# genjax-community/genjax

Measured on AMD Instinct MI355X. Metric: particle_steps_per_sec, higher is better.
Workload: dtype f32; 1 GPU; gmm_c8_d16 ImportanceK: propagate+reweight+LSE, systematic resample, gather (BASELINE.json configs[1]); k_particles_per_gpu=1048576, k_particles_total=1048576, rng_stream=flat, exchange=none

## Files before the change

### genjax_amd/csrc/gjx_resample.hip

```cpp
#include <math.h>
#include <string.h>

#include "gjx_device.h"
#include "gjx_host.h"
#include "gjx_scan.h"
#include "gjx_tile.h"

namespace gjx {

struct PickPair {
  float v;
  int32_t i;
};

GJX_DEV void pick_better(float& v, int32_t& i, float ov, int32_t oi) {
  if (ov > v || (ov == v && oi < i)) { v = ov; i = oi; }
}

template <int RNG>
__global__ __launch_bounds__(256) void k_pick_partial(const float* logw, int64_t K, int64_t offset, const float* lse,
                                                     key2 key, PickPair* partials) {
  __shared__ float rv[4];
  __shared__ int32_t ri[4];
  const float l = lse[2];
  float bv = -INFINITY;
  int32_t bi = 0x7FFFFFFF;
  for (int64_t i = (int64_t)blockIdx.x * 256 + threadIdx.x; i < K; i += (int64_t)gridDim.x * 256) {
    const uint64_t gi = (uint64_t)(offset + i);
    uint32_t bits;
    if (RNG == GJX_RNG_JAX32) {
      const key2 h = fold_in64(key, gi);
      bits = h.a ^ h.b;
    } else {
      const key2 h = fold_in64(key, gi >> 1);
      bits = (gi & 1u) ? h.b : h.a;
    }
    const float v = (logw[i] - l) + gumbel_from_bits(bits);
    pick_better(bv, bi, v, (int32_t)gi);
  }
#pragma unroll
  for (int o = 32; o > 0; o >>= 1) {
    const float ov = __shfl_xor(bv, o, 64);
    const int32_t oi = __shfl_xor(bi, o, 64);
    pick_better(bv, bi, ov, oi);
  }
  if ((threadIdx.x & 63) == 0) { rv[threadIdx.x >> 6] = bv; ri[threadIdx.x >> 6] = bi; }
  __syncthreads();
  if (threadIdx.x == 0) {
    for (int w = 1; w < 4; ++w) pick_better(bv, bi, rv[w], ri[w]);
    partials[blockIdx.x] = PickPair{bv, bi};
  }
}

__global__ __launch_bounds__(256) void k_pick_finish(const PickPair* partials, int n, PickPair* out) {
  __shared__ float rv[4];
  __shared__ int32_t ri[4];
  float bv = -INFINITY;
  int32_t bi = 0x7FFFFFFF;
  for (int t = threadIdx.x; t < n; t += 256) pick_better(bv, bi, partials[t].v, partials[t].i);
#pragma unroll
  for (int o = 32; o > 0; o >>= 1) {
    const float ov = __shfl_xor(bv, o, 64);
    const int32_t oi = __shfl_xor(bi, o, 64);
    pick_better(bv, bi, ov, oi);
  }
  if ((threadIdx.x & 63) == 0) { rv[threadIdx.x >> 6] = bv; ri[threadIdx.x >> 6] = bi; }
  __syncthreads();
  if (threadIdx.x == 0) {
    for (int w = 1; w < 4; ++w) pick_better(bv, bi, rv[w], ri[w]);
    *out = PickPair{bv, bi};
  }
}

template <int RNG>
__global__ __launch_bounds__(256) void k_trials_lse_pick(const float* logw, int64_t K, int64_t offset, key2 key, int want_pick, float log_k,
                                                        float* lse_out, int32_t* pick_out) {
  __shared__ float red[8];
  __shared__ float rv[4];
  __shared__ int32_t ri[4];
  const int64_t t = blockIdx.x;
  const float* lw = logw + t * K;
  float m = -INFINITY;
  for (int64_t i = threadIdx.x; i < K; i += 256) m = fmaxf(m, lw[i]);
  m = wave_max(m);
  if ((threadIdx.x & 63) == 0) red[threadIdx.x >> 6] = m;
  __syncthreads();
  const float bm = fmaxf(fmaxf(red[0], red[1]), fmaxf(red[2], red[3]));
  float sm = 0.0f;
  if (bm > -INFINITY)
    for (int64_t i = threadIdx.x; i < K; i += 256) sm += fast_exp(lw[i] - bm);
  sm = wave_sum(sm);
  if ((threadIdx.x & 63) == 0) red[4 + (threadIdx.x >> 6)] = sm;
  __syncthreads();
  const float bs = (red[4] + red[5]) + (red[6] + red[7]);
  const float l = bm > -INFINITY ? bm + fast_log(bs) : -INFINITY;
  if (threadIdx.x == 0) {
    float* o = lse_out + 4 * t;
    o[0] = bm; o[1] = bs; o[2] = l; o[3] = l - log_k;
  }
  if (!want_pick) return;
  float bv = -INFINITY;
  int32_t bi = 0x7FFFFFFF;
  for (int64_t i = threadIdx.x; i < K; i += 256) {
    const uint64_t gi = (uint64_t)(offset + t * K + i);
    uint32_t bits;
    if (RNG == GJX_RNG_JAX32) {
      const key2 h = fold_in64(key, gi);
      bits = h.a ^ h.b;
    } else {
      const key2 h = fold_in64(key, gi >> 1);
      bits = (gi & 1u) ? h.b : h.a;
    }
    pick_better(bv, bi, (lw[i] - l) + gumbel_from_bits(bits), (int32_t)gi);
  }
#pragma unroll
  for (int o = 32; o > 0; o >>= 1) {
    const float ov = __shfl_xor(bv, o, 64);
    const int32_t oi = __shfl_xor(bi, o, 64);
    pick_better(bv, bi, ov, oi);
  }
  if ((threadIdx.x & 63) == 0) { rv[threadIdx.x >> 6] = bv; ri[threadIdx.x >> 6] = bi; }
  __syncthreads();
  if (threadIdx.x == 0) {
    for (int w = 1; w < 4; ++w) pick_better(bv, bi, rv[w], ri[w]);
    pick_out[t] = bi == 0x7FFFFFFF ? (int32_t)(offset + t * K) : bi;
  }
}

__global__ __launch_bounds__(256) void k_wsum_blocks(const float* x, int64_t K, int is_log, const float* lse,
                                                    int n_partials, float* lse_out, float log_k_total,
                                                    uint64_t* block_sums) {
  __shared__ uint64_t red[4];
  __shared__ float fred[8];
  float sm;
  const float mx = block_ref_max(is_log, lse, n_partials, fred, &sm);
  if (is_log == 2 && lse_out && blockIdx.x == 0 && threadIdx.x == 0) {
    const float l = mx > -INFINITY ? mx + logf(sm) : -INFINITY;
    lse_out[0] = mx; lse_out[1] = sm; lse_out[2] = l; lse_out[3] = l - log_k_total;
  }
  const int64_t base = (int64_t)blockIdx.x * kScanTile + (int64_t)threadIdx.x * kScanItems;
  uint64_t s = 0;
#pragma unroll
  for (int k = 0; k < kScanItems; ++k)
    if (base + k < K) s += weight_q(x, base + k, is_log, mx);
  s = wave_sum_u64(s);
  if ((threadIdx.x & 63) == 0) red[threadIdx.x >> 6] = s;
  __syncthreads();
  if (threadIdx.x == 0) block_sums[blockIdx.x] = red[0] + red[1] + red[2] + red[3];
}

__global__ __launch_bounds__(256) void k_wscan_write(const float* x, int64_t K, int is_log, const float* lse,
                                                    int n_partials, const uint64_t* block_sums, uint64_t* cum,
                                                    uint64_t* base_total) {
  __shared__ uint64_t wsum[4];
  __shared__ uint64_t red[4];
  __shared__ float fred[8];
  const float mx = block_ref_max(is_log, lse, n_partials, fred, nullptr);
  const int64_t base = (int64_t)blockIdx.x * kScanTile + (int64_t)threadIdx.x * kScanItems;
  uint64_t pre = 0;
  for (int t = threadIdx.x; t < (int)blockIdx.x; t += 256) pre += block_sums[t];
  pre = wave_sum_u64(pre);
  if ((threadIdx.x & 63) == 0) red[threadIdx.x >> 6] = pre;
  uint64_t q[kScanItems];
  uint64_t s = 0;
#pragma unroll
  for (int k = 0; k < kScanItems; ++k) {
    q[k] = (base + k < K) ? weight_q(x, base + k, is_log, mx) : 0;
    s += q[k];
    q[k] = s;
  }
  uint64_t inc = wave_scan_u64(s);
  if ((threadIdx.x & 63) == 63) wsum[threadIdx.x >> 6] = inc;
  __syncthreads();
  uint64_t off = red[0] + red[1] + red[2] + red[3] + inc - s;
  for (int w = 0; w < (int)(threadIdx.x >> 6); ++w) off += wsum[w];
#pragma unroll
  for (int k = 0; k < kScanItems; ++k)
    if (base + k < K) cum[base + k] = off + q[k];
  if (blockIdx.x == gridDim.x - 1 && threadIdx.x == 255) {
    base_total[0] = 0;
    base_total[1] = off + s;
  }
}

GJX_DEV int64_t upper_search(const uint64_t* __restrict__ cum, int64_t K, uint64_t t) {
  int64_t lo = 0, hi = K - 1;
  while (lo < hi) {
    const int64_t mid = (lo + hi) >> 1;
    if (cum[mid] > t) hi = mid; else lo = mid + 1;
  }
  return lo;
}

GJX_DEV int64_t upper_search_in(const uint64_t* __restrict__ cum, int64_t lo, int64_t hi, uint64_t t) {
  while (lo < hi) {
    const int64_t mid = (lo + hi) >> 1;
    if (cum[mid] > t) hi = mid; else lo = mid + 1;
  }
  return lo;
}

template <bool GATHER>
__global__ __launch_bounds__(256) void k_systematic_expand(const uint64_t* __restrict__ cum, int64_t K,
                                                          const uint64_t* base_total, double u, int64_t N_total,
                                                          int64_t out_begin, int64_t n_out, int32_t* ancestors,
                                                          const float* __restrict__ src, int64_t src_stride, int rows,
                                                          float* __restrict__ dst, int64_t dst_stride,
                                                          const int64_t* range_dev = nullptr) {
  constexpr int kOwn = 8;
  if (range_dev) {
    out_begin = range_dev[0];
    const int64_t n = range_dev[1];
    n_out = n < n_out ? n : n_out;
  }
  __shared__ int n_heavy;
  __shared__ int32_t h_i[256];
  __shared__ int64_t h_lo[256], h_hi[256];
  if (threadIdx.x == 0) n_heavy = 0;
  __syncthreads();
  const int64_t i = (int64_t)blockIdx.x * 256 + threadIdx.x;
  const uint64_t base = base_total[0], total = base_total[1];
  const double step = (double)total / (double)N_total;
  const double inv_step = (double)N_total / (double)total;
  const bool in = i < K && total > 0;
  const uint64_t c_cur = in ? base + cum[i] : 0;
  const int64_t j_cur = in ? slots_below(c_cur, u, step, inv_step, total, N_total) : 0;
  int64_t j_prev = __shfl_up((long long)j_cur, 1, 64);
  uint64_t c_prev = __shfl_up((unsigned long long)c_cur, 1, 64);
  if ((threadIdx.x & 63) == 0) {
    c_prev = base + ((in && i > 0) ? cum[i - 1] : 0);
    j_prev = in ? slots_below(c_prev, u, step, inv_step, total, N_total) : 0;
  }
  if (in) {
    if (c_cur > c_prev) {
      int64_t lo = j_prev - out_begin;
      int64_t hi = j_cur - out_begin;
      lo = lo < 0 ? 0 : lo;
      hi = hi > n_out ? n_out : hi;
      if (hi - lo > kOwn) {
        const int h = atomicAdd(&n_heavy, 1);
        h_i[h] = (int32_t)i; h_lo[h] = lo; h_hi[h] = hi;
      } else if (hi > lo) {
        if (ancestors) for (int64_t j = lo; j < hi; ++j) ancestors[j] = (int32_t)i;
        if (GATHER) {
          for (int r = 0; r < rows; ++r) {
            const float v = src[(int64_t)r * src_stride + i];
            for (int64_t j = lo; j < hi; ++j) dst[(int64_t)r * dst_stride + j] = v;
          }
        }
      }
    }
  }
  __syncthreads();
  const int nh = n_heavy;
  for (int h = 0; h < nh; ++h) {
    const int32_t pi = h_i[h];
    const int64_t lo = h_lo[h], hi = h_hi[h];
    if (ancestors) for (int64_t j = lo + threadIdx.x; j < hi; j += 256) ancestors[j] = pi;
    if (GATHER) {
      for (int r = 0; r < rows; ++r) {
        const float v = src[(int64_t)r * src_stride + pi];
        for (int64_t j = lo + threadIdx.x; j < hi; j += 256) dst[(int64_t)r * dst_stride + j] = v;
      }
    }
  }
}

template <int ITEMS>
__global__ __launch_bounds__(256) void k_resample_fused(const float* __restrict__ x, int64_t K, int mode,
                                                       const float* lse, int n_partials, float* lse_out,
                                                       float log_k_total, double u, int64_t N, int32_t* ancestors,
                                                       uint64_t* cum_out, uint64_t* base_total_out,
                                                       unsigned long long* agg, unsigned* ctrl) {
  __shared__ float fred[8];
  __shared__ ScanSmem sm;
  unsigned epoch;
  const unsigned long long tag = grid_tag(ctrl, &epoch);
  const int64_t i0 = ((int64_t)blockIdx.x * 256 + threadIdx.x) * ITEMS;
  float xv[ITEMS];
#pragma unroll
  for (int k = 0; k < ITEMS; ++k) xv[k] = (i0 + k < K) ? x[i0 + k] : 0.0f;
  float sm_sum;
  const float mx = block_ref_max(mode, lse, n_partials, fred, &sm_sum);
  if (mode == 2 && lse_out && blockIdx.x == 0 && threadIdx.x == 0) {
    const float l = mx > -INFINITY ? mx + logf(sm_sum) : -INFINITY;
    lse_out[0] = mx; lse_out[1] = sm_sum; lse_out[2] = l; lse_out[3] = l - log_k_total;
  }
  tile_scan_expand<ITEMS, false>(xv, mode, mx, i0, K, u, N, ancestors, cum_out, base_total_out, agg, tag, ctrl, epoch, true, sm);
}

constexpr int kGatherMaxTiles = 1024;

template <int ITEMS>
__global__ __launch_bounds__(256) void k_resample_gather(const float* __restrict__ x, int64_t K, int mode,
                                                        const float* lse, int n_partials, float* lse_out,
                                                        float log_k_total, double u, const float* __restrict__ src,
                                                        int64_t src_stride, int rows, float* __restrict__ dst,
                                                        int64_t dst_stride, int32_t* ancestors,
                                                        unsigned long long* agg, unsigned* ctrl,
                                                        unsigned long long* timeline) {
#define GJX_STAMP(n) do { if (timeline && threadIdx.x == 0) timeline[blockIdx.x * 8 + (n)] = __builtin_amdgcn_s_memrealtime(); } while (0)
  GJX_STAMP(0);
  constexpr int TILE = 256 * ITEMS;
  __shared__ float fred[8];
  __shared__ uint64_t wsum[4];
  __shared__ uint64_t P[kGatherMaxTiles + 1];
  constexpr int CH = 3;
  __shared__ uint64_t cumL[CH * TILE];
  __shared__ uint64_t s_wtot[CH][4];
  __shared__ int s_range[2];
  unsigned epoch;
  const unsigned long long tag = grid_tag(ctrl, &epoch);
  const int nb = (int)gridDim.x;
  const int lane = threadIdx.x & 63, wid = threadIdx.x >> 6;
  const int64_t i0 = ((int64_t)blockIdx.x * 256 + threadIdx.x) * ITEMS;
  auto load_tile = [&](int64_t p0, float (&v)[ITEMS]) {
    if (ITEMS == 4 && p0 + 4 <= K) {
      const float4 q4 = *(const float4*)(x + p0);
      v[0] = q4.x; v[1] = q4.y; v[2] = q4.z; v[3] = q4.w;
    } else {
#pragma unroll
      for (int k = 0; k < ITEMS; ++k) v[k] = (p0 + k < K) ? x[p0 + k] : 0.0f;
    }
  };
  const int w0 = (int)blockIdx.x - 1;
  float xv[ITEMS], xn[2][ITEMS];
  load_tile(i0, xv);
  float sm_sum;
  const float mx = block_ref_max(mode, lse, n_partials, fred, &sm_sum);
  if (mode == 2 && lse_out && blockIdx.x == 0 && threadIdx.x == 0) {
    const float l = mx > -INFINITY ? mx + logf(sm_sum) : -INFINITY;
    lse_out[0] = mx; lse_out[1] = sm_sum; lse_out[2] = l; lse_out[3] = l - log_k_total;
  }
  uint64_t qown[ITEMS], sown = 0, incown;
  {
#pragma unroll
    for (int k = 0; k < ITEMS; ++k) { sown += (i0 + k < K) ? weight_q(xv, k, mode, mx) : 0; qown[k] = sown; }
    incown = wave_scan_u64(sown);
    if (lane == 63) { wsum[wid] = incown; s_wtot[1][wid] = incown; }
    __syncthreads();
    if (threadIdx.x == 0) grid_publish(agg, tag, wsum[0] + wsum[1] + wsum[2] + wsum[3]);
  }
  GJX_STAMP(1);
#pragma unroll
  for (int c = 0; c < 2; ++c) {
    const int tc = w0 + 2 * c;
#pragma unroll
    for (int k = 0; k < ITEMS; ++k) xn[c][k] = 0.0f;
    if (tc >= 0 && tc < nb) load_tile((int64_t)tc * TILE + (int64_t)threadIdx.x * ITEMS, xn[c]);
  }
  {
    uint64_t qn[2][ITEMS], sn[2], incn[2];
#pragma unroll
    for (int c = 0; c < 2; ++c) {
      const int tc = w0 + 2 * c;
      const bool on = tc >= 0 && tc < nb;
      const int64_t p0 = (int64_t)tc * TILE + (int64_t)threadIdx.x * ITEMS;
      sn[c] = 0;
#pragma unroll
      for (int k = 0; k < ITEMS; ++k) { sn[c] += (on && p0 + k < K) ? weight_q(xn[c], k, mode, mx) : 0; qn[c][k] = sn[c]; }
    }
#pragma unroll
    for (int c = 0; c < 2; ++c) incn[c] = wave_scan_u64(sn[c]);
    if (lane == 63) { s_wtot[0][wid] = incn[0]; s_wtot[2][wid] = incn[1]; }
    __syncthreads();
#pragma unroll
    for (int c = 0; c < 3; ++c) {
      uint64_t base = c == 1 ? incown - sown : incn[c >> 1] - sn[c >> 1];
      for (int w = 0; w < wid; ++w) base += s_wtot[c][w];
#pragma unroll
      for (int k = 0; k < ITEMS; ++k) cumL[c * TILE + threadIdx.x * ITEMS + k] = base + (c == 1 ? qown[k] : qn[c >> 1][k]);
    }
  }
  grid_gather(agg, tag, ctrl, [&](int b, unsigned long long val) { P[b + 1] = val; });
  if (threadIdx.x == 0) P[0] = 0;
  __syncthreads();
  GJX_STAMP(2);
  prefix_in_place<256>(P, nb, wsum, NoShift{});
  const uint64_t total = P[nb];
  GJX_STAMP(6);
  if (blockIdx.x == 0 && threadIdx.x == 0) {
    __hip_atomic_store(&ctrl[0], epoch + 1u, __ATOMIC_RELAXED, __HIP_MEMORY_SCOPE_AGENT);
    if (total == 0) __hip_atomic_fetch_or(&ctrl[2], kStatusZeroTotal, __ATOMIC_RELAXED, __HIP_MEMORY_SCOPE_AGENT);
  }
  int32_t anc[ITEMS];
#pragma unroll
  for (int k = 0; k < ITEMS; ++k) anc[k] = (int32_t)((i0 + k < K) ? i0 + k : 0);
  if (total > 0) {
    const double step = (double)total / (double)K;
    uint64_t T[ITEMS];
    int tile[ITEMS], kpos[ITEMS];
#pragma unroll
    for (int k = 0; k < ITEMS; ++k) {
      const int64_t j = (i0 + k < K) ? i0 + k : K - 1;
      T[k] = comb_threshold(j, u, step, total);
    }
    source_tiles<ITEMS>(P, nb, (int)blockIdx.x, T, tile);
    if (timeline) { asm volatile("" :: "v"(tile[0]), "v"(tile[ITEMS - 1])); GJX_STAMP(7); }
    if (threadIdx.x == 0) s_range[0] = tile[0];
    if (threadIdx.x == 255) s_range[1] = tile[ITEMS - 1];
    __syncthreads();
    const int tmin = s_range[0], ntiles = s_range[1] - tmin + 1;
    int pos[ITEMS];
    const uint64_t* cm[ITEMS];
    uint64_t Tr[ITEMS];
#pragma unroll
    for (int k = 0; k < ITEMS; ++k) Tr[k] = T[k] - P[tile[k]];
    if (tmin >= w0 && s_range[1] <= w0 + 2) {
      GJX_STAMP(3);
#pragma unroll
      for (int k = 0; k < ITEMS; ++k) cm[k] = cumL + (tile[k] - w0) * TILE;
      rank_in_tiles<TILE, ITEMS>(cm, Tr, pos);
#pragma unroll
      for (int k = 0; k < ITEMS; ++k) anc[k] = (int32_t)((int64_t)tile[k] * TILE + pos[k]);
    } else {
#pragma unroll
    for (int k = 0; k < ITEMS; ++k) kpos[k] = tile[k] - tmin;
    auto next_live = [&](int at) { while (at < ntiles && P[tmin + at + 1] == P[tmin + at]) ++at; return at; };
    GJX_STAMP(3);
    float nv[CH][ITEMS];
#pragma unroll
    for (int c = 0; c < CH; ++c)
      if (c < ntiles) load_tile((int64_t)(tmin + c) * TILE + (int64_t)threadIdx.x * ITEMS, nv[c]);
    for (int idx = 0; idx < ntiles;) {
      const int nidx = next_live(idx + CH);
      rescan_round<256, TILE, ITEMS, CH>(cumL, &s_wtot[0][0], [&](int c, int o, uint64_t (&q)[ITEMS]) {
        const bool on = idx + c < ntiles;
        const int64_t p0 = (int64_t)(tmin + idx + c) * TILE + o;
        if (on) {
#pragma unroll
          for (int k = 0; k < ITEMS; ++k) q[k] = (p0 + k < K) ? weight_q(nv[c], k, mode, mx) : 0;
        }
        if (nidx + c < ntiles) load_tile((int64_t)(tmin + nidx + c) * TILE + o, nv[c]);
        return on;
      }, [] {});
      bool mine[ITEMS];
#pragma unroll
      for (int k = 0; k < ITEMS; ++k) {
        mine[k] = kpos[k] >= idx && kpos[k] < idx + CH;
        cm[k] = cumL + (mine[k] ? (kpos[k] - idx) * TILE : 0);
      }
      rank_in_tiles<TILE, ITEMS>(cm, Tr, pos);
#pragma unroll
      for (int k = 0; k < ITEMS; ++k)
        if (mine[k]) anc[k] = (int32_t)((int64_t)tile[k] * TILE + pos[k]);
      idx = nidx;
    }
    }
  }
  GJX_STAMP(4);
#pragma unroll
  for (int k = 0; k < ITEMS; ++k) anc[k] = max(0, min(anc[k], (int32_t)(K - 1)));
  const bool whole = i0 + ITEMS <= K;
  if (ancestors) {
    if (ITEMS == 4 && whole) *(int4*)(ancestors + i0) = make_int4(anc[0], anc[1], anc[2], anc[3]);
    else {
#pragma unroll
      for (int k = 0; k < ITEMS; ++k) if (i0 + k < K) ancestors[i0 + k] = anc[k];
    }
  }
  const bool vec = ITEMS == 4 && whole && (dst_stride & 3) == 0 && (((uintptr_t)dst) & 15) == 0;
  if (vec) {
#pragma unroll 4
    for (int r = 0; r < rows; ++r) {
      const float* sr = src + (int64_t)r * src_stride;
      float4 v;
      v.x = sr[anc[0]]; v.y = sr[anc[ITEMS > 1 ? 1 : 0]]; v.z = sr[anc[ITEMS > 2 ? 2 : 0]]; v.w = sr[anc[ITEMS > 3 ? 3 : 0]];
      *(float4*)(dst + (int64_t)r * dst_stride + i0) = v;
    }
  } else {
#pragma unroll 4
    for (int r = 0; r < rows; ++r) {
      const float* sr = src + (int64_t)r * src_stride;
#pragma unroll
      for (int k = 0; k < ITEMS; ++k) if (i0 + k < K) dst[(int64_t)r * dst_stride + i0 + k] = sr[anc[k]];
    }
  }
  GJX_STAMP(5);
#undef GJX_STAMP
}

constexpr int kGatherTiledMaxTiles = 65536;

template <bool GATED>
__global__ __launch_bounds__(kTileQ) void k_tile_totals(const float* __restrict__ logw, int64_t K, uint64_t* S, int32_t* E, const int32_t* gate) {
  constexpr int NW = kTileQ / 64;
  if (GATED && *gate == 0) return;
  __shared__ float fred[NW];
  __shared__ uint64_t wsum[NW];
  const int64_t i = (int64_t)blockIdx.x * kTileQ + threadIdx.x;
  const float lw[1] = {i < K ? logw[i] : -INFINITY};
  uint64_t q[1], inc;
  const int e = tile_quantise<kTileQ, 1>(lw, fred, wsum, q, inc);
  if (threadIdx.x == 0) {
    const uint64_t tot = sum_partials<NW>(wsum);
    S[blockIdx.x] = tot;
    E[blockIdx.x] = tot ? e : kTileDead;
  }
}

template <int ITEMS, bool PLANNED, bool GATED>
__global__ __launch_bounds__(256) void k_resample_gather_tiled(const float* __restrict__ x, int64_t K, const uint64_t* __restrict__ S,
                                                              const int32_t* __restrict__ E, const uint64_t* __restrict__ Pg,
                                                              const int32_t* __restrict__ shg, int lse_mode, const float* lse,
                                                              int n_partials, float* lse_out, float log_k_total, double u,
                                                              const float* __restrict__ src, int64_t src_stride, int rows,
                                                              float* __restrict__ dst, int64_t dst_stride, int32_t* ancestors,
                                                              unsigned* ctrl, unsigned long long* timeline, const int32_t* gate) {
#define GJX_STAMP(n) do { if (timeline && threadIdx.x == 0) timeline[blockIdx.x * 8 + (n)] = __builtin_amdgcn_s_memrealtime(); } while (0)
  GJX_STAMP(0);
  static_assert(ITEMS == 4, "a block consumes one quantisation tile: 256 lanes x 4 slots");
  extern __shared__ __align__(16) unsigned char gt_dyn[];
  const int nt = (int)gridDim.x;
  uint64_t* const Pl = (uint64_t*)gt_dyn;
  int32_t* const Ebl = (int32_t*)(Pl + ((nt + 2) & ~1));
  __shared__ TiledSearchShared sh;
  const int64_t i0 = ((int64_t)blockIdx.x * 256 + threadIdx.x) * ITEMS;
  int32_t anc[ITEMS];
  if (GATED && *gate == 0) {
#pragma unroll
    for (int k = 0; k < ITEMS; ++k) anc[k] = (int32_t)((i0 + k < K) ? i0 + k : K - 1);
  } else
  tiled_search_tile<PLANNED>(x, K, S, E, Pg, shg, nt, (int)blockIdx.x, Pl, Ebl, sh, lse_mode, lse, n_partials, lse_out, log_k_total, u, ctrl, timeline, anc);
  GJX_STAMP(4);
  const bool whole = i0 + ITEMS <= K;
  if (ancestors) {
    if (whole) *(int4*)(ancestors + i0) = make_int4(anc[0], anc[1], anc[2], anc[3]);
    else {
#pragma unroll
      for (int k = 0; k < ITEMS; ++k) if (i0 + k < K) ancestors[i0 + k] = anc[k];
    }
  }
  const bool vec = whole && (dst_stride & 3) == 0 && (((uintptr_t)dst) & 15) == 0;
  if (vec) {
#pragma unroll 4
    for (int r = 0; r < rows; ++r) {
      const float* sr = src + (int64_t)r * src_stride;
      float4 v;
      v.x = sr[anc[0]]; v.y = sr[anc[1]]; v.z = sr[anc[2]]; v.w = sr[anc[3]];
      *(float4*)(dst + (int64_t)r * dst_stride + i0) = v;
    }
  } else {
#pragma unroll 4
    for (int r = 0; r < rows; ++r) {
      const float* sr = src + (int64_t)r * src_stride;
#pragma unroll
      for (int k = 0; k < ITEMS; ++k) if (i0 + k < K) dst[(int64_t)r * dst_stride + i0 + k] = sr[anc[k]];
    }
  }
  GJX_STAMP(5);
#undef GJX_STAMP
}

__global__ __launch_bounds__(256) void k_multinomial(const uint64_t* cum, int64_t K, const uint64_t* base_total,
                                                    key2 key, int64_t out_begin, int64_t n_out, int32_t* ancestors) {
  const int64_t j = (int64_t)blockIdx.x * 256 + threadIdx.x;
  if (j >= n_out) return;
  const uint64_t base = base_total[0], total = base_total[1];
  const key2 h = fold_in64(key, (uint64_t)(out_begin + j));
  const uint64_t r = (((uint64_t)h.a << 32) | h.b) >> 11;
  const double uj = (double)r * (1.0 / 9007199254740992.0);
  const uint64_t T = (uint64_t)(uj * (double)total);
  int32_t a = -1;
  if (K > 0) {
    const uint64_t local = cum[K - 1];
    if (T >= base && T < base + local) a = (int32_t)upper_search(cum, K, T - base);
  }
  ancestors[j] = a;
}

__global__ __launch_bounds__(256) void k_gather_rows(const float* __restrict__ src, int64_t src_stride,
                                                    const int32_t* __restrict__ anc, int64_t n_out, int rows,
                                                    float* __restrict__ dst, int64_t dst_stride) {
  const int64_t j = (int64_t)blockIdx.x * 256 + threadIdx.x;
  if (j >= n_out) return;
  const int32_t a = anc[j];
  if ((uint64_t)(int64_t)a >= (uint64_t)src_stride) return;
  for (int r = 0; r < rows; ++r) dst[(int64_t)r * dst_stride + j] = src[(int64_t)r * src_stride + a];
}


int launch_expand_planned(const uint64_t* cum, int64_t K, const gjx_shard_plan* plan_dev, double u, int64_t N_total,
                          int32_t* ancestors, int64_t anc_capacity, hipStream_t st) {
  const uint64_t* bt = reinterpret_cast<const uint64_t*>(plan_dev);
  const int64_t* range = reinterpret_cast<const int64_t*>(plan_dev) + 2;
  hipLaunchKernelGGL(k_systematic_expand<false>, dim3((unsigned)((K + 255) / 256)), dim3(256), 0, st, cum, K, bt, u, N_total,
                     (int64_t)0, anc_capacity, ancestors, (const float*)nullptr, (int64_t)0, 0, (float*)nullptr, (int64_t)0,
                     range);
  GJX_CHECK_LAUNCH("gjx_shard_resample(expand)");
  return GJX_OK;
}

struct EssArgs {
  const float* inc;
  float* W;
// ... 542 lines not shown
```

### genjax_amd/csrc/gjx_tile.h

```cpp
#pragma once
#include "gjx_device.h"
#include "gjx_scan.h"

namespace gjx {

constexpr int kSsmPersistMaxDy = 32;

GJX_DEV float load_agent(const float* p) { return __int_as_float(__hip_atomic_load((const int*)p, __ATOMIC_RELAXED, __HIP_MEMORY_SCOPE_AGENT)); }
GJX_DEV void load_agent_x4(const float* p, float (&v)[4]) {
  typedef float f4 __attribute__((ext_vector_type(4)));
  f4 r;
  asm volatile("global_load_dwordx4 %0, %1, off sc1\n\ts_waitcnt vmcnt(0)" : "=v"(r) : "v"(p) : "memory");
  v[0] = r.x; v[1] = r.y; v[2] = r.z; v[3] = r.w;
}
GJX_DEV void store_agent_x4(float* p, const float (&v)[4]) {
  typedef float f4 __attribute__((ext_vector_type(4)));
  const f4 r = {v[0], v[1], v[2], v[3]};
  asm volatile("global_store_dwordx4 %0, %1, off sc1\n\ts_nop 1" : : "v"(p), "v"(r) : "memory");
}
GJX_DEV void store_agent(float* p, float v) { __hip_atomic_store((int*)p, __float_as_int(v), __ATOMIC_RELAXED, __HIP_MEMORY_SCOPE_AGENT); }

GJX_DEV float load_scoped(const float* p, bool sys) {
  return sys ? __int_as_float(__hip_atomic_load((const int*)p, __ATOMIC_RELAXED, __HIP_MEMORY_SCOPE_SYSTEM)) : load_agent(p);
}
// ... 28 lines not shown
  h *= 0x01000193u;
  return h ^ (h >> 15);
}
template <class Tp>
GJX_DEV Tp* peer_ptr(Tp* local, long long delta) { return (Tp*)((char*)local + delta); }

template <int RNG, int DX>
struct SsmNoiseBits { uint32_t w[RNG == GJX_RNG_FLAT ? 2 * GJX_FLAT_BLOCKS(DX + (DX & 1)) : DX]; };

template <int RNG, int DX>
GJX_DEV void ssm_noise_bits(key2 skj, uint64_t gidx, SsmNoiseBits<RNG, DX>& nb) {
  if (RNG == GJX_RNG_JAX32) skj = fold_in(fold_in64(skj, gidx), 1u);
  else if (gidx >> 32) skj = threefry2x32(skj, 0xFFFFFFFFu, (uint32_t)(gidx >> 32));
  if (RNG == GJX_RNG_FLAT) {
    constexpr int NB = GJX_FLAT_BLOCKS(DX + (DX & 1));
#pragma unroll
    for (int h = 0; h < NB; ++h) {
      const key2 hh = threefry2x32(skj, (uint32_t)gidx, (1u << GJX_FLAT_SITE_SHIFT) | (uint32_t)h);
      nb.w[2 * h] = hh.a; nb.w[2 * h + 1] = hh.b;
    }
  } else {
#pragma unroll
    for (int d0 = 0; d0 < DX; ++d0) {
      const key2 h0 = threefry2x32(skj, 0u, (uint32_t)d0);
      nb.w[d0] = h0.a ^ h0.b;
    }
  }
}
template <int RNG, int DX>
GJX_DEV void ssm_noise_normals(const SsmNoiseBits<RNG, DX>& nb, float (&nz)[DX]) {
  if (RNG == GJX_RNG_FLAT) {
#pragma unroll
    for (int d0 = 0; d0 < DX; d0 += 2) {
      float n0, n1;
      box_muller(GJX_FIELD(nb.w, d0), GJX_FIELD(nb.w, d0 + 1), n0, n1);
      nz[d0] = n0;
      if (d0 + 1 < DX) nz[d0 + 1] = n1;
    }
  } else {
#pragma unroll
    for (int d0 = 0; d0 < DX; ++d0) nz[d0] = normal_from_bits_fast(nb.w[d0]);
  }
}

constexpr int kTileQ = 1024;
constexpr float kTileScale = 536870912.0f;
constexpr int kTileDead = -524288;
constexpr float kLog2e = 1.44269504f;

GJX_DEV int tile_exponent(float tile_max) {
  if (!(tile_max > -INFINITY)) return kTileDead;
  const float t = ceilf(tile_max * kLog2e);
  return t < -524287.0f ? -524287 : (t > 524287.0f ? 524287 : (int)t);
}
GJX_DEV uint64_t tile_q(float lw, int e) {
  if (e == kTileDead) return 0;
  float w = __builtin_amdgcn_exp2f(fmaf(lw, kLog2e, -(float)e));
  w = w > 0.0f ? w : 0.0f;
  w = w < 1.0f ? w : 1.0f;
  return (uint64_t)(uint32_t)(w * kTileScale);
}
GJX_DEV unsigned long long tile_granule(unsigned long long tag, int e, uint64_t S) {
  return (tag << 60) | ((unsigned long long)(unsigned)(e - kTileDead) << 40) | (S & ((1ull << 40) - 1));
}
GJX_DEV void tile_granule_unpack(unsigned long long v, uint64_t& S, int& e) {
  S = v & ((1ull << 40) - 1);
  e = S ? (int)((v >> 40) & 0xFFFFFu) + kTileDead : kTileDead;
}
constexpr int kGranulePad = 8;


template <int THREADS, int ITEMS>
GJX_DEV int tile_quantise(const float (&lw)[ITEMS], float* red_m, uint64_t* red_q, uint64_t (&q)[ITEMS], uint64_t& inc) {
  constexpr int NW = THREADS / 64;
  const int lane = threadIdx.x & 63, wid = threadIdx.x >> 6;
  float m = lw[0];
#pragma unroll
  for (int k = 1; k < ITEMS; ++k) m = fmaxf(m, lw[k]);
  const float wm = wave_max(m);
  if (lane == 0) red_m[wid] = wm;
  __syncthreads();
  float bm = red_m[0];
#pragma unroll
  for (int w = 1; w < NW; ++w) bm = fmaxf(bm, red_m[w]);
  const int e = tile_exponent(bm);
  uint64_t s = 0;
#pragma unroll
  for (int k = 0; k < ITEMS; ++k) { q[k] = tile_q(lw[k], e); s += q[k]; }
  inc = wave_scan_u64(s);
  const uint64_t wt = lane63_u64(inc);
  if (lane == 0) red_q[wid] = wt;
  __syncthreads();
  return e;
}
template <int NW>
GJX_DEV uint64_t sum_partials(const uint64_t* w) {
  uint64_t t = 0;
#pragma unroll
  for (int k = 0; k < NW; ++k) t += w[k];
  return t;
}

struct NoShift {};
template <class A, class B> struct SameType { static constexpr bool value = false; };
template <class A> struct SameType<A, A> { static constexpr bool value = true; };
template <int THREADS, class ShiftOf>
GJX_DEV void prefix_in_place(uint64_t* P, int n, uint64_t* wave_partials, ShiftOf shift_of) {
  static_assert(THREADS >= 64 && (THREADS & (THREADS - 1)) == 0, "whole waves, a power of two");
  const int lane = threadIdx.x & 63, wid = threadIdx.x >> 6;
  const int t = THREADS == 64 ? lane : (int)threadIdx.x;
  const int per = (n + THREADS - 1) >> __builtin_ctz((unsigned)THREADS);
  const int e0 = t * per < n ? t * per : n, e1 = (e0 + per) < n ? (e0 + per) : n;
  uint64_t loc = 0;
  for (int e = e0; e < e1; ++e) {
    uint64_t g = P[e + 1];
    if constexpr (!SameType<ShiftOf, NoShift>::value) {
      const int sh = shift_of(e);
      g = sh < 64 ? g >> sh : 0;
      P[e + 1] = g;
    }
    loc += g;
  }
  const uint64_t inc = wave_scan_u64(loc);
  uint64_t run = inc - loc;
  if constexpr (THREADS > 64) {
    if (lane == 63) wave_partials[wid] = inc;
    __syncthreads();
    for (int w = 0; w < wid; ++w) run += wave_partials[w];
  }
  for (int e = e0; e < e1; ++e) { run += P[e + 1]; P[e + 1] = run; }
  if constexpr (THREADS > 64) __syncthreads();
}
template <class ShiftOf>
GJX_DEV void prefix_in_place_wave(uint64_t* P, int n, ShiftOf shift_of) { prefix_in_place<64>(P, n, nullptr, shift_of); }

template <class Val, class Out>
GJX_DEV uint64_t block_scan_chunked(int n, uint64_t* wsum, Val val, Out out) {
  const int lane = threadIdx.x & 63, wid = threadIdx.x >> 6;
  uint64_t carry = 0;
  for (int b0 = 0; b0 < n; b0 += 1024) {
    const int b = b0 + threadIdx.x;
    const uint64_t inc = wave_scan_u64(b < n ? val(b) : 0ull);
    __syncthreads();
    if (lane == 63) wsum[wid] = inc;
    __syncthreads();
    uint64_t base = carry, tot = 0;
    for (int w = 0; w < 16; ++w) { if (w < wid) base += wsum[w]; tot += wsum[w]; }
    if (b < n) out(b, base + inc);
    carry += tot;
  }
  return carry;
}

template <int ITEMS>
GJX_DEV void source_tiles(const uint64_t* P, int n, int own, const uint64_t (&T)[ITEMS], int (&tile)[ITEMS]) {
  const int wlo = own - 4 < 0 ? 0 : (own - 4 > n - 8 ? (n - 8 < 0 ? 0 : n - 8) : own - 4);
  uint64_t Pw[9];
#pragma unroll
  for (int k = 0; k < 9; ++k) Pw[k] = P[wlo + k < n ? wlo + k : n];
  if (T[0] >= Pw[0] && T[ITEMS - 1] < Pw[8]) {
#pragma unroll
    for (int k = 0; k < ITEMS; ++k) {
      int tl = wlo;
#pragma unroll
      for (int w = 1; w < 8; ++w) tl += Pw[w] <= T[k] ? 1 : 0;
      tile[k] = tl;
    }
    return;
  }
#pragma unroll
  for (int k = 0; k < ITEMS; ++k) tile[k] = 0;
  auto descend = [&](int k0, int k1) {
    for (int sft = 1 << (31 - __builtin_clz((unsigned)n)); sft >= 1; sft >>= 1) {
      const int pa = tile[k0] + sft, pb = tile[k1] + sft;
      if (pa <= n - 1 && P[pa] <= T[k0]) tile[k0] = pa;
      if (k1 != k0 && pb <= n - 1 && P[pb] <= T[k1]) tile[k1] = pb;
    }
  };
  descend(0, ITEMS - 1);
  if constexpr (ITEMS > 2) {
    if (tile[0] == tile[ITEMS - 1]) {
#pragma unroll
      for (int k = 1; k < ITEMS - 1; ++k) tile[k] = tile[0];
    } else {
#pragma unroll
      for (int k = 1; k < ITEMS - 1; k += 2) descend(k, k + 1 < ITEMS - 1 ? k + 1 : k);
    }
  }
}
GJX_DEV int source_tile(const uint64_t* P, int n, int own, uint64_t T) {
  const uint64_t T1[1] = {T};
  int tile[1];
  source_tiles<1>(P, n, own, T1, tile);
  return tile[0];
}

template <int TILE, int N>
GJX_DEV void rank_in_tiles(const uint64_t* (&cm)[N], const uint64_t (&r)[N], int (&pos)[N]) {
#pragma unroll
  for (int k = 0; k < N; ++k) pos[k] = 0;
#pragma unroll
  for (int q = TILE >> 2; q >= 1; q >>= 2) {
#pragma unroll
    for (int k = 0; k < N; ++k) {
      const uint64_t pa = cm[k][pos[k] + q - 1], pb = cm[k][pos[k] + 2 * q - 1], pc = cm[k][pos[k] + 3 * q - 1];
      pos[k] += (pa <= r[k] ? q : 0) + (pb <= r[k] ? q : 0) + (pc <= r[k] ? q : 0);
    }
  }
}
template <int TILE>
GJX_DEV int rank_in_tile(const uint64_t* cm, uint64_t r) {
  const uint64_t* cm1[1] = {cm};
  const uint64_t r1[1] = {r};
  int pos[1];
  rank_in_tiles<TILE, 1>(cm1, r1, pos);
  return pos[0];
}

template <int THREADS, int TILE, int ITEMS, int CPT, class Fill, class Mid>
GJX_DEV void rescan_round(uint64_t* cum, uint64_t* wtot, Fill fill, Mid mid) {
  constexpr int WPT = TILE / (64 * ITEMS), NW = THREADS / 64;
  const int lane = threadIdx.x & 63, wid = threadIdx.x >> 6;
  const int tl0 = NW == WPT ? 0 : (wid / WPT) * CPT, part = NW == WPT ? wid : wid % WPT, o = (part * 64 + lane) * ITEMS;
  uint64_t qi[CPT][ITEMS], sacc[CPT], inc[CPT];
  bool on[CPT];
#pragma unroll
  for (int c = 0; c < CPT; ++c) {
    uint64_t q[ITEMS];
    sacc[c] = 0; inc[c] = 0;
    on[c] = fill(tl0 + c, o, q);
    if (!on[c]) continue;
#pragma unroll
    for (int k = 0; k < ITEMS; ++k) { sacc[c] += q[k]; qi[c][k] = sacc[c]; }
  }
#pragma unroll
  for (int c = 0; c < CPT; ++c) if (on[c]) inc[c] = wave_scan_u64(sacc[c]);
  if constexpr (WPT > 1) {
    if (lane == 63) {
#pragma unroll
      for (int c = 0; c < CPT; ++c) if (on[c]) wtot[(tl0 + c) * WPT + part] = inc[c];
    }
    __syncthreads();
  }
  mid();
#pragma unroll
  for (int c = 0; c < CPT; ++c) {
    if (!on[c]) continue;
    uint64_t base = inc[c] - sacc[c];
    if constexpr (WPT > 1) for (int w = 0; w < part; ++w) base += wtot[(tl0 + c) * WPT + w];
#pragma unroll
    for (int k = 0; k < ITEMS; ++k) cum[(tl0 + c) * TILE + o + k] = base + qi[c][k];
  }
  __syncthreads();
}

GJX_DEV int64_t tiled_lookup(const uint64_t* P, const int32_t* sh, const uint64_t* cq, int nt, int64_t K, uint64_t T) {
  int lo = 0, hi = nt - 1;
  while (lo < hi) {
    const int mid = (lo + hi) >> 1;
    if (P[mid + 1] > T) hi = mid; else lo = mid + 1;
  }
  const uint64_t r = (T - P[lo]) << sh[lo];
  const uint64_t* cm = cq + (int64_t)lo * kTileQ;
  const int64_t left = K - (int64_t)lo * kTileQ;
  int l2 = 0, h2 = (int)(left < kTileQ ? left : kTileQ) - 1;
  while (l2 < h2) {
    const int mid = (l2 + h2) >> 1;
    if (cm[mid] > r) h2 = mid; else l2 = mid + 1;
  }
  return (int64_t)lo * kTileQ + l2;
}

struct TiledSearchShared {
  float fred[8];
  uint64_t wsum[4];
  uint64_t cumL[3 * 1024];
  uint64_t s_wtot[3][4];
  int s_range[2];
};

template <bool PLANNED, bool LIVE = false>
GJX_DEV void tiled_search_tile(const float* __restrict__ x, int64_t K, const uint64_t* __restrict__ S, const int32_t* __restrict__ E,
                               const uint64_t* __restrict__ Pg, const int32_t* __restrict__ shg, const int nt, const int tix, uint64_t* const Pl,
                               int32_t* const Ebl, TiledSearchShared& sh, int lse_mode, const float* lse, int n_partials, float* lse_out,
                               float log_k_total, double u, unsigned* ctrl, unsigned long long* timeline, int32_t (&anc)[4],
                               unsigned long long rtag = 0ull) {
  static_assert(!(PLANNED && LIVE), "the live form reduces the granules itself");
#define GJX_STAMP(n) do { if (timeline && threadIdx.x == 0) timeline[tix * 8 + (n)] = __builtin_amdgcn_s_memrealtime(); } while (0)
  constexpr int ITEMS = 4, TILE = 256 * ITEMS, CH = 3;
  const uint64_t* const P = PLANNED ? Pg : Pl;
  const int32_t* const Eb = PLANNED ? E : Ebl;
  const int lane = threadIdx.x & 63, wid = threadIdx.x >> 6;
  const int64_t i0 = ((int64_t)tix * 256 + threadIdx.x) * ITEMS;
  auto load_tile = [&](int64_t p0, float (&v)[ITEMS]) {
    if constexpr (LIVE) {
#pragma unroll
      for (int k = 0; k < ITEMS; ++k) v[k] = (p0 + k < K) ? load_agent(x + p0 + k) : -INFINITY;
    } else if (p0 + 4 <= K) {
      const float4 q4 = *(const float4*)(x + p0);
      v[0] = q4.x; v[1] = q4.y; v[2] = q4.z; v[3] = q4.w;
    } else {
#pragma unroll
      for (int k = 0; k < ITEMS; ++k) v[k] = (p0 + k < K) ? x[p0 + k] : -INFINITY;
    }
  };
  const int w0 = tix - 1;
  float xw[CH][ITEMS];
  auto load_window = [&]() {
#pragma unroll
    for (int c = 0; c < CH; ++c) {
#pragma unroll
      for (int k = 0; k < ITEMS; ++k) xw[c][k] = -INFINITY;
      const int tc = w0 + c;
      if (tc >= 0 && tc < nt) load_tile((int64_t)tc * TILE + (int64_t)threadIdx.x * ITEMS, xw[c]);
    }
  };
  if constexpr (!LIVE) load_window();
  int Emax = 0;
  if constexpr (!PLANNED) {
  float em = (float)kTileDead;
  if constexpr (LIVE) {
    unsigned budget = (ctrl && (__hip_atomic_load(&ctrl[2], __ATOMIC_RELAXED, __HIP_MEMORY_SCOPE_AGENT) & kStatusPollTimeout)) ? 0u : kPollBudget;
    for (int b = threadIdx.x; b < nt; b += 256) {
      unsigned long long v = __hip_atomic_load((const unsigned long long*)&S[(size_t)b * kGranulePad], __ATOMIC_RELAXED, __HIP_MEMORY_SCOPE_AGENT);
      while ((v >> 60) != rtag && budget) {
        --budget;
        __builtin_amdgcn_s_sleep(1);
        v = __hip_atomic_load((const unsigned long long*)&S[(size_t)b * kGranulePad], __ATOMIC_RELAXED, __HIP_MEMORY_SCOPE_AGENT);
      }
      if ((v >> 60) != rtag) { if (ctrl) __hip_atomic_fetch_or(&ctrl[2], kStatusPollTimeout, __ATOMIC_RELAXED, __HIP_MEMORY_SCOPE_AGENT); v = 0; }
      uint64_t sv;
      int e;
      tile_granule_unpack(v, sv, e);
      Pl[b + 1] = sv;
      Ebl[b] = e;
      em = fmaxf(em, (float)e);
    }
    __syncthreads();
    load_window();
  } else {
  for (int b = threadIdx.x; b < nt; b += 256) {
    const uint64_t sv = S[b];
    const int e = sv ? E[b] : kTileDead;
    Pl[b + 1] = sv;
    Ebl[b] = e;
    em = fmaxf(em, (float)e);
  }
  }
  em = wave_max(em);
  if (lane == 0) sh.fred[wid] = em;
  if (threadIdx.x == 0) Pl[0] = 0;
  __syncthreads();
  Emax = (int)fmaxf(fmaxf(sh.fred[0], sh.fred[1]), fmaxf(sh.fred[2], sh.fred[3]));
  GJX_STAMP(1);
  prefix_in_place<256>(Pl, nt, sh.wsum, [&](int b) { return Emax - Ebl[b]; });
  }
  auto shift_of = [&](int t) { return PLANNED ? shg[t] : Emax - Eb[t]; };
  const uint64_t total = P[nt];
  GJX_STAMP(2);
  if (tix == 0) {
    if (lse_mode == 2 && lse_out) {
      float sm_sum;
      const float mx = LIVE ? block_ref_max_live(lse, n_partials, sh.fred, &sm_sum) : block_ref_max(2, lse, n_partials, sh.fred, &sm_sum);
      if (threadIdx.x == 0) {
        const float l = mx > -INFINITY ? mx + logf(sm_sum) : -INFINITY;
        lse_out[0] = mx; lse_out[1] = sm_sum; lse_out[2] = l; lse_out[3] = l - log_k_total;
      }
    }
    if (threadIdx.x == 0 && total == 0 && ctrl) __hip_atomic_fetch_or(&ctrl[2], kStatusZeroTotal, __ATOMIC_RELAXED, __HIP_MEMORY_SCOPE_AGENT);
  }
#pragma unroll
  for (int k = 0; k < ITEMS; ++k) anc[k] = (int32_t)((i0 + k < K) ? i0 + k : K - 1);
  if (total > 0) {
    const double step = (double)total / (double)K;
    uint64_t T[ITEMS];
    int tile[ITEMS];
#pragma unroll
    for (int k = 0; k < ITEMS; ++k) {
      const int64_t j = (i0 + k < K) ? i0 + k : K - 1;
      T[k] = comb_threshold(j, u, step, total);
    }
    source_tiles<ITEMS>(P, nt, tix, T, tile);
    uint64_t Tr[ITEMS];
#pragma unroll
    for (int k = 0; k < ITEMS; ++k) Tr[k] = (T[k] - P[tile[k]]) << shift_of(tile[k]);
    if (threadIdx.x == 0) sh.s_range[0] = tile[0];
    if (threadIdx.x == 255) sh.s_range[1] = tile[ITEMS - 1];
    __syncthreads();
    const int tmin = sh.s_range[0], tmax = sh.s_range[1];
    GJX_STAMP(3);
    const bool windowed = tmin >= w0 && tmax <= w0 + 2;
    if (windowed) {
      rescan_round<256, TILE, ITEMS, CH>(sh.cumL, &sh.s_wtot[0][0], [&](int c, int, uint64_t (&q)[ITEMS]) {
        const int tc = w0 + c;
        if (tc < tmin || tc > tmax) return false;
#pragma unroll
        for (int k = 0; k < ITEMS; ++k) q[k] = tile_q(xw[c][k], Eb[tc]);
        return true;
      }, [] {});
#pragma unroll
      for (int k = 0; k < ITEMS; ++k) anc[k] = (int32_t)((int64_t)tile[k] * TILE + rank_in_tile<TILE>(sh.cumL + (tile[k] - w0) * TILE, Tr[k]));
    } else {
      const int ntiles = tmax - tmin + 1;
      auto next_live = [&](int at) { while (at < ntiles && P[tmin + at + 1] == P[tmin + at]) ++at; return at; };
      for (int idx = 0; idx < ntiles;) {
        const int nidx = next_live(idx + CH);
        __syncthreads();
        rescan_round<256, TILE, ITEMS, CH>(sh.cumL, &sh.s_wtot[0][0], [&](int c, int o, uint64_t (&q)[ITEMS]) {
          if (idx + c >= ntiles) return false;
          const int tsrc = tmin + idx + c;
          float nv[ITEMS];
          load_tile((int64_t)tsrc * TILE + o, nv);
#pragma unroll
          for (int k = 0; k < ITEMS; ++k) q[k] = tile_q(nv[k], Eb[tsrc]);
          return true;
        }, [] {});
#pragma unroll
        for (int k = 0; k < ITEMS; ++k) {
          const int kp = tile[k] - tmin;
          if (kp >= idx && kp < idx + CH) anc[k] = (int32_t)((int64_t)tile[k] * TILE + rank_in_tile<TILE>(sh.cumL + (kp - idx) * TILE, Tr[k]));
        }
        idx = nidx;
      }
    }
#pragma unroll
    for (int k = 0; k < ITEMS; ++k) anc[k] = anc[k] < K ? anc[k] : (int32_t)(K - 1);
  }
#undef GJX_STAMP
}

}
```

Baseline: 18.60 billion particle-steps/s.

## Skip full tile-prefix scan via windowed partial sums and reuse sorted rank windows

In the resample-gather kernel, each block now accumulates the global total and the sum of tile weights below its 8-tile source window during the grid gather, builds a local prefix over that window, and locates source tiles from it. The full block-wide prefix_in_place over all tile sums only runs on the fallback path when thresholds leave the window. A new rank_in_tiles_sorted exploits the sortedness of a thread's thresholds: after one binary search it loads a small 16-byte-aligned window of cumulative sums and counts within it for later items, falling back to a full search only when the window is exhausted. This removes a block-level scan and synchronisations plus repeated LDS binary searches, at the cost of extra registers and more complex control flow.

New measurement: 18.81 billion particle-steps/s (median of 6 runs). +1.1%, better.

```diff
diff --git a/genjax_amd/csrc/gjx_resample.hip b/genjax_amd/csrc/gjx_resample.hip
--- a/genjax_amd/csrc/gjx_resample.hip
+++ b/genjax_amd/csrc/gjx_resample.hip
@@ -1,3 +1,4 @@
+#include <limits.h>
 #include <math.h>
 #include <string.h>
 
@@ -304,9 +305,10 @@
   constexpr int TILE = 256 * ITEMS;
   __shared__ float fred[8];
   __shared__ uint64_t wsum[4];
+  __shared__ uint64_t s_sums[8];
   __shared__ uint64_t P[kGatherMaxTiles + 1];
   constexpr int CH = 3;
-  __shared__ uint64_t cumL[CH * TILE];
+  __shared__ __align__(16) uint64_t cumL[CH * TILE];
   __shared__ uint64_t s_wtot[CH][4];
   __shared__ int s_range[2];
   unsigned epoch;
@@ -372,13 +374,21 @@
       for (int k = 0; k < ITEMS; ++k) cumL[c * TILE + threadIdx.x * ITEMS + k] = base + (c == 1 ? qown[k] : qn[c >> 1][k]);
     }
   }
-  grid_gather(agg, tag, ctrl, [&](int b, unsigned long long val) { P[b + 1] = val; });
+  const int wlo = source_window_start(nb, (int)blockIdx.x);
+  uint64_t below = 0, total = 0;
+  grid_gather(agg, tag, ctrl, [&](int b, unsigned long long val) {
+    P[b + 1] = val;
+    total += val;
+    below += b < wlo ? val : 0;
+  });
+  below = wave_sum_u64(below);
+  total = wave_sum_u64(total);
+  if (lane == 0) { s_sums[wid] = below; s_sums[4 + wid] = total; }
   if (threadIdx.x == 0) P[0] = 0;
   __syncthreads();
+  below = sum_partials<4>(s_sums);
+  total = sum_partials<4>(s_sums + 4);
   GJX_STAMP(2);
-  prefix_in_place<256>(P, nb, wsum, NoShift{});
-  const uint64_t total = P[nb];
-  GJX_STAMP(6);
   if (blockIdx.x == 0 && threadIdx.x == 0) {
     __hip_atomic_store(&ctrl[0], epoch + 1u, __ATOMIC_RELAXED, __HIP_MEMORY_SCOPE_AGENT);
     if (total == 0) __hip_atomic_fetch_or(&ctrl[2], kStatusZeroTotal, __ATOMIC_RELAXED, __HIP_MEMORY_SCOPE_AGENT);
@@ -395,25 +405,50 @@
       const int64_t j = (i0 + k < K) ? i0 + k : K - 1;
       T[k] = comb_threshold(j, u, step, total);
     }
+    uint64_t Tr[ITEMS];
+    uint64_t Pw[9];
+    Pw[0] = below;
+#pragma unroll
+    for (int w = 1; w < 9; ++w) Pw[w] = Pw[w - 1] + (wlo + w <= nb ? P[wlo + w] : 0);
+    GJX_STAMP(6);
+#pragma unroll
+    for (int k = 0; k < ITEMS; ++k) {
+      tile[k] = wlo;
+      uint64_t lo = Pw[0];
+#pragma unroll
+      for (int w = 1; w < 8; ++w) {
+        const bool past = Pw[w] <= T[k];
+        tile[k] += past ? 1 : 0;
+        lo = past ? Pw[w] : lo;
+      }
+      Tr[k] = T[k] - lo;
+    }
+    if (timeline) { asm volatile("" :: "v"(tile[0]), "v"(tile[ITEMS - 1])); GJX_STAMP(7); }
+    if (threadIdx.x == 0) s_range[0] = T[0] >= Pw[0] ? tile[0] : INT_MIN;
+    if (threadIdx.x == 255) s_range[1] = T[ITEMS - 1] < Pw[8] ? tile[ITEMS - 1] : INT_MAX;
+    __syncthreads();
+    int tmin = s_range[0], tmax = s_range[1];
+    const bool windowed = tmin >= w0 && tmax <= w0 + 2;
+    int pos[ITEMS];
+    const uint64_t* cm[ITEMS];
+    if (windowed) {
+      GJX_STAMP(3);
+#pragma unroll
+      for (int k = 0; k < ITEMS; ++k) cm[k] = cumL + (tile[k] - w0) * TILE;
+      if constexpr (ITEMS > 1) rank_in_tiles_sorted<TILE, ITEMS>(cm, Tr, pos);
+      else rank_in_tiles<TILE, ITEMS>(cm, Tr, pos);
+#pragma unroll
+      for (int k = 0; k < ITEMS; ++k) anc[k] = (int32_t)((int64_t)tile[k] * TILE + pos[k]);
+    } else {
+    prefix_in_place<256>(P, nb, wsum, NoShift{});
     source_tiles<ITEMS>(P, nb, (int)blockIdx.x, T, tile);
-    if (timeline) { asm volatile("" :: "v"(tile[0]), "v"(tile[ITEMS - 1])); GJX_STAMP(7); }
+#pragma unroll
+    for (int k = 0; k < ITEMS; ++k) Tr[k] = T[k] - P[tile[k]];
     if (threadIdx.x == 0) s_range[0] = tile[0];
     if (threadIdx.x == 255) s_range[1] = tile[ITEMS - 1];
     __syncthreads();
-    const int tmin = s_range[0], ntiles = s_range[1] - tmin + 1;
-    int pos[ITEMS];
-    const uint64_t* cm[ITEMS];
-    uint64_t Tr[ITEMS];
-#pragma unroll
-    for (int k = 0; k < ITEMS; ++k) Tr[k] = T[k] - P[tile[k]];
-    if (tmin >= w0 && s_range[1] <= w0 + 2) {
-      GJX_STAMP(3);
-#pragma unroll
-      for (int k = 0; k < ITEMS; ++k) cm[k] = cumL + (tile[k] - w0) * TILE;
-      rank_in_tiles<TILE, ITEMS>(cm, Tr, pos);
-#pragma unroll
-      for (int k = 0; k < ITEMS; ++k) anc[k] = (int32_t)((int64_t)tile[k] * TILE + pos[k]);
-    } else {
+    tmin = s_range[0]; tmax = s_range[1];
+    const int ntiles = tmax - tmin + 1;
 #pragma unroll
     for (int k = 0; k < ITEMS; ++k) kpos[k] = tile[k] - tmin;
     auto next_live = [&](int at) { while (at < ntiles && P[tmin + at + 1] == P[tmin + at]) ++at; return at; };
@@ -440,7 +475,8 @@
         mine[k] = kpos[k] >= idx && kpos[k] < idx + CH;
         cm[k] = cumL + (mine[k] ? (kpos[k] - idx) * TILE : 0);
       }
-      rank_in_tiles<TILE, ITEMS>(cm, Tr, pos);
+      if constexpr (ITEMS > 1) rank_in_tiles_sorted<TILE, ITEMS>(cm, Tr, mine, pos);
+      else rank_in_tiles<TILE, ITEMS>(cm, Tr, pos);
 #pragma unroll
       for (int k = 0; k < ITEMS; ++k)
         if (mine[k]) anc[k] = (int32_t)((int64_t)tile[k] * TILE + pos[k]);
diff --git a/genjax_amd/csrc/gjx_tile.h b/genjax_amd/csrc/gjx_tile.h
--- a/genjax_amd/csrc/gjx_tile.h
+++ b/genjax_amd/csrc/gjx_tile.h
@@ -204,9 +204,12 @@
   return carry;
 }
 
+GJX_DEV int source_window_start(int n, int own) {
+  return own - 4 < 0 ? 0 : (own - 4 > n - 8 ? (n - 8 < 0 ? 0 : n - 8) : own - 4);
+}
 template <int ITEMS>
 GJX_DEV void source_tiles(const uint64_t* P, int n, int own, const uint64_t (&T)[ITEMS], int (&tile)[ITEMS]) {
-  const int wlo = own - 4 < 0 ? 0 : (own - 4 > n - 8 ? (n - 8 < 0 ? 0 : n - 8) : own - 4);
+  const int wlo = source_window_start(n, own);
   uint64_t Pw[9];
 #pragma unroll
   for (int k = 0; k < 9; ++k) Pw[k] = P[wlo + k < n ? wlo + k : n];
@@ -268,6 +271,51 @@
   rank_in_tiles<TILE, 1>(cm1, r1, pos);
   return pos[0];
 }
+constexpr int kRankWalk = 12;
+template <int TILE, int N>
+GJX_DEV void rank_in_tiles_sorted(const uint64_t* (&cm)[N], const uint64_t (&r)[N], const bool (&on)[N], int (&pos)[N]) {
+  typedef uint64_t u64x2 __attribute__((ext_vector_type(2)));
+  constexpr int W = kRankWalk;
+  static_assert(N > 1 && W % 2 == 0 && W <= TILE && TILE % 2 == 0, "an even window inside the tile");
+  const uint64_t* acm = cm[0];
+  bool aon = on[0];
+  int base = 0;
+  u64x2 win[W / 2] = {};
+  auto anchor_at = [&](int at) {
+    const int even = at & ~1;
+    base = even > TILE - W ? TILE - W : even;
+#pragma unroll
+    for (int j = 0; j < W / 2; ++j) win[j] = ((const u64x2*)(acm + base))[j];
+  };
+  pos[0] = 0;
+  if (on[0]) {
+    pos[0] = rank_in_tile<TILE>(cm[0], r[0]);
+    anchor_at(pos[0]);
+  }
+#pragma unroll
+  for (int k = 1; k < N; ++k) {
+    bool full = on[k];
+    pos[k] = 0;
+    if (on[k] && aon && cm[k] == acm) {
+      int cnt = 0;
+#pragma unroll
+      for (int j = 0; j < W / 2; ++j) cnt += (win[j].x <= r[k] ? 1 : 0) + (win[j].y <= r[k] ? 1 : 0);
+      pos[k] = base + cnt;
+      full = cnt == W && base + W < TILE;
+    }
+    if (full) {
+      pos[k] = rank_in_tile<TILE>(cm[k], r[k]);
+      if (k + 1 < N) { acm = cm[k]; aon = true; anchor_at(pos[k]); }
+    }
+  }
+}
+template <int TILE, int N>
+GJX_DEV void rank_in_tiles_sorted(const uint64_t* (&cm)[N], const uint64_t (&r)[N], int (&pos)[N]) {
+  bool on[N];
+#pragma unroll
+  for (int k = 0; k < N; ++k) on[k] = true;
+  rank_in_tiles_sorted<TILE, N>(cm, r, on, pos);
+}
 
 template <int THREADS, int TILE, int ITEMS, int CPT, class Fill, class Mid>
 GJX_DEV void rescan_round(uint64_t* cum, uint64_t* wtot, Fill fill, Mid mid) {
@@ -326,7 +374,7 @@
 struct TiledSearchShared {
   float fred[8];
   uint64_t wsum[4];
-  uint64_t cumL[3 * 1024];
+  alignas(16) uint64_t cumL[3 * 1024];
   uint64_t s_wtot[3][4];
   int s_range[2];
 };
@@ -450,8 +498,13 @@
         for (int k = 0; k < ITEMS; ++k) q[k] = tile_q(xw[c][k], Eb[tc]);
         return true;
       }, [] {});
-#pragma unroll
-      for (int k = 0; k < ITEMS; ++k) anc[k] = (int32_t)((int64_t)tile[k] * TILE + rank_in_tile<TILE>(sh.cumL + (tile[k] - w0) * TILE, Tr[k]));
+      const uint64_t* cm[ITEMS];
+      int pos[ITEMS];
+#pragma unroll
+      for (int k = 0; k < ITEMS; ++k) cm[k] = sh.cumL + (tile[k] - w0) * TILE;
+      rank_in_tiles_sorted<TILE, ITEMS>(cm, Tr, pos);
+#pragma unroll
+      for (int k = 0; k < ITEMS; ++k) anc[k] = (int32_t)((int64_t)tile[k] * TILE + pos[k]);
     } else {
       const int ntiles = tmax - tmin + 1;
       auto next_live = [&](int at) { while (at < ntiles && P[tmin + at + 1] == P[tmin + at]) ++at; return at; };
@@ -467,11 +520,19 @@
           for (int k = 0; k < ITEMS; ++k) q[k] = tile_q(nv[k], Eb[tsrc]);
           return true;
         }, [] {});
+        const uint64_t* cm[ITEMS];
+        bool mine[ITEMS];
+        int pos[ITEMS];
 #pragma unroll
         for (int k = 0; k < ITEMS; ++k) {
           const int kp = tile[k] - tmin;
-          if (kp >= idx && kp < idx + CH) anc[k] = (int32_t)((int64_t)tile[k] * TILE + rank_in_tile<TILE>(sh.cumL + (kp - idx) * TILE, Tr[k]));
+          mine[k] = kp >= idx && kp < idx + CH;
+          cm[k] = sh.cumL + (mine[k] ? (kp - idx) * TILE : 0);
         }
+        rank_in_tiles_sorted<TILE, ITEMS>(cm, Tr, mine, pos);
+#pragma unroll
+        for (int k = 0; k < ITEMS; ++k)
+          if (mine[k]) anc[k] = (int32_t)((int64_t)tile[k] * TILE + pos[k]);
         idx = nidx;
       }
     }
```
